# christofw/multipitch_architectures

Measured on NVIDIA B200. Metric: audio_seconds_per_second, higher is better.
Workload: dtype fp16

## Files before the change

include/mpa.h:

```cpp
#ifndef MPA_H_
#define MPA_H_

#include <stddef.h>
#include <stdint.h>

#ifdef __cplusplus
extern "C" {
#endif

#define MPA_OK 0
#define MPA_ERR_ARG (-1)
#define MPA_ERR_ARCH (-2)
#define MPA_ERR_CUDA (-3)
#define MPA_ERR_WORKSPACE (-4)

#define MPA_ACT_NONE 0
#define MPA_ACT_LRELU 1
#define MPA_ACT_RELU 2
#define MPA_ACT_SIGMOID 3

#define MPA_FMT_F16 0
#define MPA_FMT_BF16 1
#define MPA_FMT_F16X3 2

// ... 112 lines not shown
int mpa_conv_tc_pack_weights_dev(const float* w_dev, void* packed_dev, int Cin, int Cout, int KH, int KW, int fmt, int J,
                                 int transpose_flip, int Cout_total, int co0, void* stream);
typedef struct mpa_pack_job {
  const float* w;
  void* packed;
  int Cin, Cout, KH, KW, fmt, J, transpose_flip, Cout_total, co0;
  int split, C0;
} mpa_pack_job;
int mpa_conv_tc_pack_weights_split_dev(const float* w_dev, void* packed_dev, int Cin, int Cout, int KH, int KW, int fmt, int J,
                                       int transpose_flip, int Cout_total, int co0, int split, int C0, void* stream);
size_t mpa_conv_tc_pack_table_bytes(int n_jobs);
int mpa_conv_tc_pack_table_build(const mpa_pack_job* jobs, int n_jobs, void* table_host);
int mpa_conv_tc_pack_weights_multi(const void* table_dev, int n_jobs, int n_blocks, void* stream);
size_t mpa_conv_tc_ring_packed_bytes(int Cin, int Cout, int KH, int KW, int J);
int mpa_conv_tc_ring_pack_weights(const float* w_host, void* packed_host, int Cin, int Cout, int KH, int KW, int fmt, int J);
int mpa_conv_tc_pool_f16(const mpa_conv_tc_desc* desc, void* stream);
int mpa_pool_time_res_cp8(const void* y_cp8, const void* res_cp8, void* out_cp8, int n_patches, int C, int T, int F,
                          int pitch, int pf, int pt, int k, int fmt, int ncs_y, int ncs_res, int ncs_out, void* stream);
int mpa_maxpool2x2_cp8(const void* in_cp8, void* out_cp8, int n, int C, int T, int F, int pitch_in, int pf_in,
                       int pt_in, int ncs_in, int pitch_out, int pf_out, int pt_out, int ncs_out, int fmt, void* stream);
int mpa_upsample2x_cp8(const void* low_cp8, void* out_cp8, int n, int C, int Tl, int Fl, int pitch_l, int pf_l, int pt_l,
                       int ncs_l, int Ts, int Fs, int pitch_s, int pf_s, int pt_s, int ncs_out, int fmt, void* stream);
int mpa_nchw_to_cp8(const float* x, void* out_cp8, int B, int C, int T, int F, int pitch, int pf, int pt, int fmt,
                    int ncs_out, void* stream);
int mpa_nchw_to_cp8_strided(const float* x, void* out_cp8, int B, int C, int T, int Fs, int F, int stride, int offset, int pitch,
                            int pf, int pt, int fmt, int ncs_out, void* stream);
int mpa_cp8_to_nchw(const void* in_cp8, float* out, int B, int C, int T, int F, int pitch, int pf, int pt, int fmt,
                    int ncs_in, void* stream);

int mpa_head_tail_cp8(const void* x_cp8, const float* w3, const float* b3, const float* w40, const float* b40,
                      const float* w43, const float* b43, float* out, int B, int C1, int T, int Fo, int C2, int C3,
// ... 167 lines not shown
```

multipitch_architectures_b200/csrc/conv_tc.cu:

```cuda
#include "common.cuh"
#include <cuda.h>
#include <cuda_fp16.h>
#include <vector>
#include <string.h>
#include <math.h>

namespace mpa {

constexpr int kStageMMAs = 8;
constexpr int kATileBytes = 2 * 128 * 16;
constexpr int kAStageBytes = kStageMMAs * kATileBytes;
constexpr int kMaxAStages = 5;
constexpr int kNumBStages = 2;
constexpr int kMaxBStages = 8;
constexpr int kThreads = 320;
constexpr int kMaxRingS = 24;
constexpr int kMaxRingB = 8;
constexpr int kMaxGrid = 160;
constexpr int kEpiPitch = 40;
constexpr unsigned long long kWaitTimeoutNs = 4000000000ull;

struct ConvTcParams {
  const uint8_t* in_edge;
  const uint8_t* in_stream;
// ... 140 lines not shown

struct UnitInfo {
  int b, seg, t0;
  bool first_in_seg;
};
__device__ __forceinline__ UnitInfo decode_unit(const ConvTcParams& p, int u) {
  UnitInfo ui;
  ui.b = u / p.groups_per_patch;
  int g = u - ui.b * p.groups_per_patch;
  ui.seg = 0;
  if (g >= p.seg_groups[0]) { g -= p.seg_groups[0]; ui.seg = 1; }
  ui.t0 = p.y_lo[ui.seg] + g * p.J * p.R;
  ui.first_in_seg = (g == 0);
  return ui;
}
__device__ __forceinline__ void unit_range(const ConvTcParams& p, int& u_begin, int& u_end, int& u_first_real) {
  const long long U = p.n_units;
  u_first_real = (int)(U * blockIdx.x / gridDim.x);
  u_end = (int)(U * (blockIdx.x + 1) / gridDim.x);
  u_begin = u_first_real;
  if (p.pool && u_first_real < u_end && !decode_unit(p, u_first_real).first_in_seg) u_begin = u_first_real - 1;
}
__device__ __forceinline__ const uint8_t* in_row_ptr(const ConvTcParams& p, int b, int row, long long& chunk_stride) {
  if (row < p.in_e || row >= p.T - p.in_e) {
    const int idx = row < p.in_e ? row : row - (p.T - 2 * p.in_e);
    chunk_stride = p.in_edge_chunk_stride;
    return p.in_edge + (long long)b * p.in_edge_patch_stride + (long long)idx * p.P * 16;
  }
  chunk_stride = p.in_stream_chunk_stride;
  return p.in_stream + ((long long)b * p.in_stream_patch_rows + row) * p.P * 16;
}
__device__ __forceinline__ uint8_t* out_row_ptr(const ConvTcParams& p, int b, int row, long long& chunk_stride) {
  if (row < p.out_e || row >= p.T - p.out_e) {
    const int idx = row < p.out_e ? row : row - (p.T - 2 * p.out_e);
    chunk_stride = p.out_edge_chunk_stride;
    return p.out_edge + (long long)b * p.out_edge_patch_stride + (long long)idx * p.P * 16;
// ... 28 lines not shown
    }
  } else {
    __half2* cm = reinterpret_cast<__half2*>(&c);
    const __half2* rm = reinterpret_cast<const __half2*>(&r);
#pragma unroll
    for (int e = 0; e < 4; ++e) {
      float2 a = __half22float2(cm[e]), b2 = __half22float2(rm[e]);
      cm[e] = __floats2half2_rn(a.x + b2.x, a.y + b2.y);
    }
  }
  return c;
}

template <bool X3>
__device__ __forceinline__ void epilogue_role(const ConvTcParams& p, uint32_t tmem_base, uint16_t* epi_smem, uint64_t* acc_full, uint64_t* acc_empty,
                                              int u_begin, int u_end, int u_first_real) {
  const int warp = threadIdx.x >> 5, lane = threadIdx.x & 31;
  {
    const int quad = warp & 3;
    const int m = quad * 32 + lane;
    const int j = m / p.Cout, co = m - j * p.Cout;
    const bool row_valid = (j < p.J);
    const float bias = row_valid ? p.bias[co] : 0.f;
    const float inv_scale = (X3 && row_valid) ? p.inv_scale[co] : 1.f;
    constexpr int n_parts = X3 ? 2 : 1;
    const float act_slope = p.act == MPA_ACT_NONE ? 1.f : p.act == MPA_ACT_RELU ? 0.f : p.act_param;
    const bool fast_act = p.act != MPA_ACT_SIGMOID && act_slope >= 0.f && act_slope <= 1.f;
    const int NCoP = n_parts * p.NCo;
    const bool staged = ((p.Cout & 7) == 0);
    const int ewarp = warp - 2;
    const int ehalf = ewarp >> 2;
    const int etid = threadIdx.x - 64;
    uint16_t* stile = epi_smem + ewarp * (32 * kEpiPitch);
    int grp_j[4], grp_plane[4];
#pragma unroll
    for (int k = 0; k < 4; ++k) {
      const int mg = quad * 32 + k * 8;
      grp_j[k] = mg / p.Cout;
      grp_plane[k] = (mg - grp_j[k] * p.Cout) >> 3;
    }
    const size_t plane_elems = (p.out_mode == 0) ? (size_t)p.TP_out * p.P * 8 : (p.out_mode == 2) ? (size_t)p.TP_out * p.P2 * 8 : (size_t)p.T_out * p.F_out * 8;
    const int row_pitch = (p.out_mode == 0) ? p.P : (p.out_mode == 2) ? p.P2 : p.F_out;
    const size_t ring_row_bytes = (size_t)NCoP * p.P * 16;
    uint8_t* ring_cta = p.pool ? p.ring + (size_t)blockIdx.x * 2 * p.J * ring_row_bytes : nullptr;
    uint32_t k_unit = 0;
    for (int u = u_begin; u < u_end; ++u, ++k_unit) {
      const UnitInfo ui = decode_unit(p, u);
      const int b = ui.b, t0 = ui.t0;
      const int y_hi = p.y_hi[ui.seg];
      const int t = t0 + j;
      const uint32_t buf = k_unit & 1u, acc_par = (k_unit >> 1) & 1u;
      uint8_t* ring_bank = p.pool ? ring_cta + (size_t)(k_unit & 1u) * p.J * ring_row_bytes : nullptr;
      mbar_wait(&acc_full[buf], acc_par);
      tc_fence_after();
      uint16_t* out_b = p.out + (size_t)b * p.out_patch_stride;
      for (int c0 = ehalf * 32; c0 < p.N; c0 += 64) {
        const int n = c0 + lane;
        int rr = 0, nn = n;
        if (p.R > 1) { rr = n / p.P; nn = n - rr * p.P; }
        int fo = nn - p.pf;
// ... 156 lines not shown
              *reinterpret_cast<uint4*>(op) = c;
            } else {
              long long ocs;
              uint8_t* op = out_row_ptr(p, b, tz, ocs);
              *reinterpret_cast<uint4*>(op + (long long)ck * ocs + (size_t)(p.pf + f) * 16) = c;
            }
          }
        }
        epi_bar_sync();
      }
    }
  }
}

template <bool X3>
__global__ void __launch_bounds__(kThreads, 1) conv_tc_kernel(const __grid_constant__ ConvTcParams p) {
  extern __shared__ __align__(1024) uint8_t smem[];
  const int slab_plane_bytes = p.slab_px * 16;
  const int bstage_bytes = min(p.G, p.NC) * slab_plane_bytes + p.bpad;
  const int kNumAStages = p.a_stages;
  uint8_t* a_smem = smem;
  uint8_t* b_smem = smem + kNumAStages * kAStageBytes;
  const int nbs = p.b_stages;
  uint64_t* bars = reinterpret_cast<uint64_t*>(b_smem + nbs * bstage_bytes);
  uint64_t* a_full = bars;
  uint64_t* a_empty = bars + kMaxAStages;
  uint64_t* b_full = bars + 2 * kMaxAStages;
  uint64_t* b_empty = b_full + kMaxBStages;
  uint64_t* acc_full = b_empty + kMaxBStages;
  uint64_t* acc_empty = acc_full + 2;
  uint32_t* tmem_slot = reinterpret_cast<uint32_t*>(acc_empty + 2);
// ... 21 lines not shown
    for (int i = threadIdx.x; i < nbs * bstage_bytes / 16; i += kThreads) reinterpret_cast<uint4*>(b_smem)[i] = make_uint4(0, 0, 0, 0);
    asm volatile("fence.proxy.async.shared::cta;" ::: "memory");
  }
  if (warp == 1) {
    asm volatile("tcgen05.alloc.cta_group::1.sync.aligned.shared::cta.b32 [%0], %1;" ::"r"(smem_u32(tmem_slot)), "r"(512u));
    asm volatile("tcgen05.relinquish_alloc_permit.cta_group::1.sync.aligned;");
  }
  tc_fence_before();
  __syncthreads();
  tc_fence_after();
  const uint32_t tmem_base = *tmem_slot;

  const int ph = p.KH / 2, pw = p.KW / 2;
  const int rows_in = p.KH + p.J - 1;
  constexpr int n_parts = X3 ? 2 : 1;
  int u_begin, u_end, u_first_real;
  unit_range(p, u_begin, u_end, u_first_real);

  if (warp == 0) {
    {
      int a_stage = 0, b_stage = 0;
      uint32_t a_phase = 0, b_phase = 0;
      if (lane == 0 && p.resident && u_begin < u_end) {
        const int spr = (p.mmas_per_row + kStageMMAs - 1) / kStageMMAs;
        for (int r = 0; r < rows_in; ++r)
          for (int m0 = 0; m0 < p.mmas_per_row; m0 += kStageMMAs) {
            const int nm = min(kStageMMAs, p.mmas_per_row - m0), idx = r * spr + m0 / kStageMMAs;
            mbar_expect_tx(&a_full[idx], (uint32_t)(nm * kATileBytes));
            bulk_g2s(a_smem + idx * kAStageBytes, p.w + ((size_t)r * p.mmas_per_row + m0) * kATileBytes, (uint32_t)(nm * kATileBytes), &a_full[idx]);
          }
      }
      __syncwarp();
      for (int u = u_begin; u < u_end; ++u) {
        const UnitInfo ui = decode_unit(p, u);
        for (int r = 0; r < rows_in; ++r) {
          const int row = ui.t0 - ph + r;
          if (p.R == 1 && (row < 0 || row >= p.T)) continue;
          for (int part = 0; part < n_parts; ++part) {
           for (int gi = 0; gi < p.n_groups; ++gi) {
            const int planes = min(p.G, p.NC - gi * p.G);
            uint8_t* dst = b_smem + b_stage * bstage_bytes;
            if (p.tma) {
              if (lane == 0) {
                mbar_wait(&b_empty[b_stage], b_phase ^ 1);
                mbar_expect_tx(&b_full[b_stage], (uint32_t)(min(p.G, p.NC) * slab_plane_bytes));
                asm volatile(
                    "cp.async.bulk.tensor.4d.shared::cluster.global.tile.mbarrier::complete_tx::bytes [%0], [%1, {%2, %3, %4, %5}], [%6];" ::"r"(
// ... 40 lines not shown
            const int n_tiles = (X3 && part == 0) ? 2 * p.mmas_per_row : (gi == p.n_groups - 1 ? p.mmas_per_row : (gi + 1) * (p.G / 2) * p.KW) - q0;
            const uint8_t* wrow = p.w + ((size_t)r * p.tiles_per_row + (part ? 2 * p.mmas_per_row : 0) + q0) * kATileBytes;
            for (int m0 = 0; m0 < n_tiles; m0 += kStageMMAs) {
              const int nm = min(kStageMMAs, n_tiles - m0);
              if (lane == 0) {
                mbar_wait(&a_empty[a_stage], a_phase ^ 1);
                mbar_expect_tx(&a_full[a_stage], (uint32_t)(nm * kATileBytes));
                bulk_g2s(a_smem + a_stage * kAStageBytes, wrow + (size_t)m0 * kATileBytes, (uint32_t)(nm * kATileBytes), &a_full[a_stage]);
              }
              if (++a_stage == kNumAStages) { a_stage = 0; a_phase ^= 1; }
            }
           }
          }
        }
      }
    }
    __syncwarp();
  } else if (warp == 1) {
    {
      const uint32_t tmem_u = __shfl_sync(0xffffffffu, tmem_base, 0);
      int a_stage = 0, b_stage = 0;
      uint32_t a_phase = 0, b_phase = 0;
      constexpr uint32_t kDescHi = (128u >> 4) | (1u << 14);
      constexpr uint32_t kALoFixed = ((128u * 16u) >> 4) << 16;
      const uint32_t asm16 = smem_u32(a_smem) >> 4, bsm16 = smem_u32(b_smem) >> 4, bst16 = (uint32_t)bstage_bytes >> 4;
      uint32_t k_unit = 0;
      const int spr = (p.mmas_per_row + kStageMMAs - 1) / kStageMMAs;
      if (p.resident && u_begin < u_end)
        for (int i = 0; i < rows_in * spr; ++i) mbar_wait(&a_full[i], 0);
      for (int u = u_begin; u < u_end; ++u, ++k_unit) {
        const UnitInfo ui = decode_unit(p, u);
        const uint32_t buf = k_unit & 1u, acc_par = (k_unit >> 1) & 1u;
        mbar_wait(&acc_empty[buf], acc_par ^ 1);
        tc_fence_after();
        const uint32_t tmem_d = tmem_u + buf * 256;
        uint32_t accum = 0;
        for (int r = 0; r < rows_in; ++r) {
          const int row = ui.t0 - ph + r;
          if (p.R == 1 && (row < 0 || row >= p.T)) continue;
          for (int part = 0; part < n_parts; ++part) {
          for (int gi = 0; gi < p.n_groups; ++gi) {
          const int q0 = gi * (p.G / 2) * p.KW;
          const int n_tiles = (X3 && part == 0) ? 2 * p.mmas_per_row : (gi == p.n_groups - 1 ? p.mmas_per_row : (gi + 1) * (p.G / 2) * p.KW) - q0;
          mbar_wait(&b_full[b_stage], b_phase);
// ... 20 lines not shown
              if (!p.resident) tc_commit(&a_empty[a_stage]);
            }
            __syncwarp();
            accum = 1;
            if (!p.resident && ++a_stage == kNumAStages) { a_stage = 0; a_phase ^= 1; }
          }
          if (elect_one_sync()) tc_commit(&b_empty[b_stage]);
          __syncwarp();
          if (++b_stage == nbs) { b_stage = 0; b_phase ^= 1; }
          }
          }
        }
        if (elect_one_sync()) tc_commit(&acc_full[buf]);
        __syncwarp();
      }
    }
    __syncwarp();
  } else {
    epilogue_role<X3>(p, tmem_base, epi_smem, acc_full, acc_empty, u_begin, u_end, u_first_real);
  }
  tc_fence_before();
  __syncthreads();
  if (warp == 1) {
    tc_fence_after();
    asm volatile("tcgen05.dealloc.cta_group::1.sync.aligned.b32 %0, %1;" ::"r"(tmem_base), "r"(512u));
  }
}

template <int Q, int BSTEP>
__device__ __forceinline__ void issue_tile(uint32_t tmem_d, uint32_t a_lo, uint32_t a_hi, uint32_t b_lo, uint32_t b_hi, uint32_t idesc, uint32_t first) {
  tc_mma_f16(tmem_d, ((uint64_t)a_hi << 32) | (uint64_t)a_lo, ((uint64_t)b_hi << 32) | (uint64_t)b_lo, idesc, first ? 0u : 1u);
#pragma unroll
  for (int q = 1; q < Q; ++q)
    tc_mma_f16(tmem_d, ((uint64_t)a_hi << 32) | (uint64_t)(a_lo + (uint32_t)q * 16u), ((uint64_t)b_hi << 32) | (uint64_t)(b_lo + (uint32_t)(q * BSTEP)), idesc, 1u);
}
__device__ __forceinline__ void ring_group(const ConvTcParams& p, int g, int& Q, int& planes, int& chunk0) {
  if (g < p.NC / 2) { Q = p.KW; planes = 2; chunk0 = 2 * g; }
  else { Q = (p.KW + 1) / 2; planes = 1; chunk0 = p.NC - 1; }
}

__global__ void __launch_bounds__(kThreads, 1) conv_tc_ring_kernel(const ConvTcParams p) {
  extern __shared__ __align__(1024) uint8_t smem[];
  const int slab_plane_bytes = p.slab_px * 16;
  const int bstage_bytes = 2 * slab_plane_bytes;
  const int S = p.ring_S, NB = p.ring_nb;
  uint8_t* ring = smem;
  uint8_t* b_smem = smem + p.ring_b_off;
  uint64_t* bars = reinterpret_cast<uint64_t*>(smem + p.ring_bar_off);
  uint64_t* w_full = bars;
  uint64_t* w_empty = bars + kMaxRingS;
  uint64_t* b_full = bars + 2 * kMaxRingS;
  uint64_t* b_empty = b_full + kMaxRingB;
  uint64_t* acc_full = b_empty + kMaxRingB;
  uint64_t* acc_empty = acc_full + 2;
  uint32_t* tmem_slot = reinterpret_cast<uint32_t*>(acc_empty + 2);
  uint32_t* btab = reinterpret_cast<uint32_t*>(smem + p.btab_off);
// ... 8 lines not shown
  }
  if (warp == 1) {
    asm volatile("tcgen05.alloc.cta_group::1.sync.aligned.shared::cta.b32 [%0], %1;" ::"r"(smem_u32(tmem_slot)), "r"(512u));
    asm volatile("tcgen05.relinquish_alloc_permit.cta_group::1.sync.aligned;");
  }
  tc_fence_before();
  __syncthreads();
  tc_fence_after();
  const uint32_t tmem_base = *tmem_slot;

  const int ph = p.KH / 2, pw = p.KW / 2;
  const int rows_in = p.KH + p.J - 1;
  const int NG = (p.NC + 1) / 2;
  const int G8 = p.Cout >> 3;
  const int n_kh = p.KH + 2 * (p.J - 1);
  int u_begin, u_end, u_first_real;
  unit_range(p, u_begin, u_end, u_first_real);

  if (warp == 0) {
    if (lane == 0) {
      uint32_t n_piece = 0;
      int b_stage = 0;
      uint32_t b_phase = 0;
      for (int u = u_begin; u < u_end; ++u) {
        const UnitInfo ui = decode_unit(p, u);
        const int r_first = max(0, ph - ui.t0), r_last = min(rows_in - 1, p.T - 1 - ui.t0 + ph);
        size_t g_off = 0;
        for (int g = 0; g < NG; ++g) {
          int Q, planes, chunk0;
          ring_group(p, g, Q, planes, chunk0);
          const uint32_t row_bytes = (uint32_t)Q * 256u;
          const uint8_t* wg = p.w + g_off;
          for (int kh = r_first - (p.J - 1); kh <= r_last; ++kh, ++n_piece) {
            const int pos = S - 1 - (int)(n_piece % (uint32_t)S);
            const uint32_t round = n_piece / (uint32_t)S;
            const bool mirror = pos <= p.J - 2;
            mbar_wait(&w_empty[pos], (round & 1u) ^ 1u);
            const bool mir = mirror;
// ... 12 lines not shown
            if (kh >= r_first) {
              const int row = ui.t0 - ph + kh;
              mbar_wait(&b_empty[b_stage], b_phase ^ 1);
              mbar_expect_tx(&b_full[b_stage], (uint32_t)(planes * slab_plane_bytes));
              long long cs;
              const uint8_t* bsrc = in_row_ptr(p, ui.b, row, cs) - pw * 16 + (long long)chunk0 * cs;
              uint8_t* bdst = b_smem + b_stage * bstage_bytes;
              for (int c = 0; c < planes; ++c)
                bulk_g2s(bdst + c * slab_plane_bytes, bsrc + (long long)c * cs, (uint32_t)slab_plane_bytes, &b_full[b_stage]);
              if (++b_stage == NB) { b_stage = 0; b_phase ^= 1; }
            }
          }
          g_off += (size_t)n_kh * G8 * row_bytes;
        }
      }
    }
    __syncwarp();
  } else if (warp == 1) {
    {
      const uint32_t tmem_u = __shfl_sync(0xffffffffu, tmem_base, 0);
      uint32_t n_piece = 0;
      int b_stage = 0;
      uint32_t b_phase = 0;
      const uint32_t kDescHiB = (128u >> 4) | (1u << 14);
      const uint32_t kDescHiA = ((uint32_t)p.ring_sbo >> 4) | (1u << 14);
      constexpr uint32_t kALoFixed = (128u >> 4) << 16;
      const uint32_t ring16 = smem_u32(ring) >> 4, ps16 = (uint32_t)p.ring_ps >> 4;
      const uint32_t bsm16 = smem_u32(b_smem) >> 4, bst16 = (uint32_t)bstage_bytes >> 4;
      const uint32_t plane16 = (uint32_t)slab_plane_bytes >> 4;
      uint32_t k_unit = 0;
      for (int u = u_begin; u < u_end; ++u, ++k_unit) {
        const UnitInfo ui = decode_unit(p, u);
        const int r_first = max(0, ph - ui.t0), r_last = min(rows_in - 1, p.T - 1 - ui.t0 + ph);
        const uint32_t buf = k_unit & 1u, acc_par = (k_unit >> 1) & 1u;
        mbar_wait(&acc_empty[buf], acc_par ^ 1);
        tc_fence_after();
        const uint32_t tmem_d = tmem_u + buf * 256;
        uint32_t first = 1;
        for (int g = 0; g < NG; ++g) {
          const bool pair = g < p.NC / 2;
          const int Q = pair ? p.KW : (p.KW + 1) / 2;
          const uint32_t b_lo_fixed = pair ? (plane16 << 16) : (1u << 16);
          for (int kh = r_first - (p.J - 1); kh <= r_last; ++kh, ++n_piece) {
            const int pos = S - 1 - (int)(n_piece % (uint32_t)S);
            mbar_wait(&w_full[pos], (n_piece / (uint32_t)S) & 1u);
// ... 13 lines not shown
                             p.idesc, (q == 0 && first) ? 0u : 1u);
              }
              tc_commit(&b_empty[b_stage]);
              tc_commit(&w_empty[S - 1 - (int)(n_old % (uint32_t)S)]);
              if (kh == r_last)
                for (int jj = p.J - 2; jj >= 0; --jj) tc_commit(&w_empty[S - 1 - (int)((n_piece - (uint32_t)jj) % (uint32_t)S)]);
            }
            __syncwarp();
            first = 0;
            if (++b_stage == NB) { b_stage = 0; b_phase ^= 1; }
          }
        }
        if (elect_one_sync()) tc_commit(&acc_full[buf]);
        __syncwarp();
      }
    }
  } else {
    epilogue_role<false>(p, tmem_base, epi_smem, acc_full, acc_empty, u_begin, u_end, u_first_real);
  }
  tc_fence_before();
  __syncthreads();
  if (warp == 1) {
    tc_fence_after();
    asm volatile("tcgen05.dealloc.cta_group::1.sync.aligned.b32 %0, %1;" ::"r"(tmem_base), "r"(512u));
  }
}

static inline int j_blocks(int Cout) { return Cout >= 128 ? 1 : 128 / Cout; }
static inline int mmas_per_row(int NC, int KW) { return (NC / 2) * KW + ((NC & 1) ? (KW + 1) / 2 : 0); }

static inline uint16_t f32_to_f16_rne(float f) {
  uint32_t x;
  memcpy(&x, &f, 4);
// ... 706 lines not shown
              const int co = g8 * 8 + row;
              for (int e = 0; e < 8; ++e) {
                const int ci = c * 8 + e;
                if (ci >= Cin) continue;
                const float wv = w[(((size_t)co * Cin + ci) * KH + kh) * KW + df];
                o[g_off + ((((size_t)khi * G8 + g8) * Q + q) * 2 + ks) * 64 + row * 8 + e] = fmt == MPA_FMT_BF16 ? f32_to_bf16_rne(wv) : f32_to_f16_rne(wv);
              }
            }
          }
    }
    g_off += (size_t)n_kh * G8 * Q * 128;
  }
  return MPA_OK;
}

static int launch_conv_tc(ConvTcParams& p, int Cin, cudaStream_t stream, int* grid_out) {
  p.mmas_per_row = mmas_per_row(p.NC, p.KW);
  p.slab_px = (p.N + 2 * (p.KW / 2) + 1 + 7) / 8 * 8;
  if (p.R < 1) p.R = 1;
  if (p.Rs < 1) p.Rs = 1;
  p.tma = 0;
  p.tma_c0 = 0;
  const bool tma_ok = !p.x3 && !p.ring_on && p.in_e == p.T && tensor_map_encoder();
  if (tma_ok && (p.Rs > 1 || p.R > 1) && p.KW == 1) {
    p.tma = 1;
    p.slab_px = p.N;
  } else if (tma_ok && p.R == 1 && p.Rs == 1 && p.NC >= 2 && p.slab_px <= 128) {
    p.tma = 2;
    p.tma_c0 = -2 * (p.KW / 2);
  }
  p.bpad = p.tma ? 128 : 0;
  size_t smem = 0;
  if (p.x3) {
    MPA_REQUIRE(!p.ring_on, "conv_tc: the ring main loop has no split-precision variant");
    MPA_REQUIRE((p.Cout & 7) == 0, "conv_tc(fp16x3): Cout must be a multiple of 8 (got %d)", p.Cout);
    p.inv_scale = (const float*)(p.w + (size_t)3 * (p.KH + p.J - 1) * p.mmas_per_row * kATileBytes);
  }
  if (p.ring_on) {
// ... 73 lines not shown
  MPA_REQUIRE(smem <= 227 * 1024, "conv_tc: needs %zu B of shared memory (Cin=%d pitch=%d)", smem, Cin, p.P);
  {
    static unsigned char flags_tile[64], flags_ring[64], flags_x3[64];
    cudaError_t e = p.ring_on ? opt_in_max_smem(conv_tc_ring_kernel, flags_ring)
                    : p.x3    ? opt_in_max_smem(conv_tc_kernel<true>, flags_x3)
                              : opt_in_max_smem(conv_tc_kernel<false>, flags_tile);
    if (e != cudaSuccess) {
      set_error("conv_tc: cudaFuncSetAttribute: %s", cudaGetErrorString(e));
      return MPA_ERR_CUDA;
    }
  }
  int dev = 0, sms = 148;
  cudaGetDevice(&dev);
  cudaDeviceGetAttribute(&sms, cudaDevAttrMultiProcessorCount, dev);
  if (sms > kMaxGrid) sms = kMaxGrid;
  const int grid = p.n_units < sms ? p.n_units : sms;
  if (grid_out) *grid_out = grid;
  if (p.ring_on)
    conv_tc_ring_kernel<<<grid, kThreads, smem, stream>>>(p);
  else if (p.x3)
    conv_tc_kernel<true><<<grid, kThreads, smem, stream>>>(p);
  else
    conv_tc_kernel<false><<<grid, kThreads, smem, stream>>>(p);
  MPA_CHECK_LAUNCH("conv_tc");
  return MPA_OK;
}

int mpa_conv_tc_f16(const void* in_cp8, const void* w_packed, const float* bias, void* out, int out_mode, int sub_stride,
                    int sub_offset, int n_patches, int Cin, int Cout, int T, int F, int KH, int KW, int pitch, int pf, int pt,
                    long long in_patch_stride_rows, int in_nc_stride, int out_nc_stride, int J, int row0, int n_rows, int act,
                    float act_param, int fmt, void* stream) {
  MPA_CHECK_ARCH();
  MPA_REQUIRE(in_cp8 && w_packed && bias && out && n_patches > 0, "conv_tc: null argument");
  MPA_REQUIRE(Cout > 0 && Cout <= 128 && Cin > 0, "conv_tc: Cout must be in 1..128 (got %d)", Cout);
  MPA_REQUIRE((KH & 1) && (KW & 1), "conv_tc: odd kernel sizes only");
  MPA_REQUIRE(fmt == MPA_FMT_F16 || fmt == MPA_FMT_BF16 || fmt == MPA_FMT_F16X3, "conv_tc: fmt must be MPA_FMT_F16, MPA_FMT_BF16 or MPA_FMT_F16X3");
  const bool x3 = fmt == MPA_FMT_F16X3;
  MPA_REQUIRE(!x3 || in_patch_stride_rows <= 0, "conv_tc(fp16x3): the streaming input goes through mpa_conv_tc_pool_f16");
// ... 65 lines not shown
    p.R = 256 / pitch;
    p.Rs = p.J;
    p.N = p.R * pitch;
  }
  p.n_seg = 1;
  p.y_lo[0] = p.z_lo[0] = row0;
  p.y_hi[0] = p.z_hi[0] = row0 + p.T_out;
  p.seg_groups[0] = (p.T_out + p.J * p.R - 1) / (p.J * p.R);
  p.seg_groups[1] = 0;
  p.groups_per_patch = p.seg_groups[0];
  p.n_units = n_patches * p.groups_per_patch;
  p.act = act;
  p.act_param = act_param;
  const uint32_t f = (fmt == MPA_FMT_BF16) ? 1u : 0u;
  p.idesc = (1u << 4) | (f << 7) | (f << 10) | ((uint32_t)(p.N >> 3) << 17) | ((uint32_t)(128 >> 4) << 24);
  return launch_conv_tc(p, Cin, (cudaStream_t)stream, nullptr);
}

size_t mpa_conv_tc_pool_workspace(int Cout, int pitch, int J) {
  if (Cout <= 0 || Cout > 128 || pitch <= 0) return 0;
  if (J <= 0) J = j_blocks(Cout);
  return (size_t)kMaxGrid * 2 * J * ((Cout + 7) / 8) * pitch * 16;
}

size_t mpa_conv_tc_pool_workspace_fmt(int Cout, int pitch, int J, int fmt) {
  return mpa_conv_tc_pool_workspace(Cout, pitch, J) * (fmt == MPA_FMT_F16X3 ? 2 : 1);
}

int mpa_conv_tc_pool_f16(const mpa_conv_tc_desc* d, void* stream) {
  MPA_CHECK_ARCH();
  MPA_REQUIRE(d && d->w_packed && d->bias && d->workspace && d->n_patches > 0, "conv_tc_pool: null argument");
  MPA_REQUIRE(d->Cout > 0 && d->Cout <= 64 && (d->Cout & 7) == 0 && d->Cin > 0, "conv_tc_pool: Cout must be a multiple of 8, <= 64 (got %d)", d->Cout);
  MPA_REQUIRE((d->KH & 1) && (d->KW & 1), "conv_tc_pool: odd kernel sizes only");
  MPA_REQUIRE(d->fmt == MPA_FMT_F16 || d->fmt == MPA_FMT_BF16 || d->fmt == MPA_FMT_F16X3, "conv_tc_pool: fmt must be MPA_FMT_F16, MPA_FMT_BF16 or MPA_FMT_F16X3");
  const int pitch = d->pitch, KW = d->KW, F = d->F, pf = d->pf, T = d->T;
  MPA_REQUIRE(pitch >= 16 && pitch <= 256 && pitch % 16 == 0, "conv_tc_pool: row pitch %d must be a multiple of 16 (<= 256)", pitch);
  MPA_REQUIRE(pf >= KW / 2 && pitch - F >= KW / 2 && pitch >= pf + F, "conv_tc_pool: pitch %d / left pad %d too small for F=%d KW=%d", pitch, pf, F, KW);
  const int J = d->J > 0 ? d->J : j_blocks(d->Cout);
  MPA_REQUIRE(J >= 2 && J * d->Cout <= 128, "conv_tc_pool: needs 2 <= J and J*Cout <= 128");
  MPA_REQUIRE(d->in_e == T || (d->in_e >= 0 && 2 * d->in_e <= T), "conv_tc_pool: in_e must be T or <= T/2");
  MPA_REQUIRE(d->out_e == T || (d->out_e >= 0 && 2 * d->out_e <= T), "conv_tc_pool: out_e must be T or <= T/2");
  MPA_REQUIRE((d->in_e == 0 || d->in_edge) && (d->in_e == T || d->in_stream), "conv_tc_pool: missing input plane");
  MPA_REQUIRE((d->out_e == 0 || d->out_edge) && (d->out_e == T || d->out_stream), "conv_tc_pool: missing output plane");
  MPA_REQUIRE(d->n_seg == 1 || d->n_seg == 2, "conv_tc_pool: 1 or 2 row segments");
  ConvTcParams p;
  memset(&p, 0, sizeof(p));
  p.in_edge = (const uint8_t*)d->in_edge;
  p.in_stream = (const uint8_t*)d->in_stream;
  p.in_edge_patch_stride = d->in_edge_patch_stride;
  p.in_edge_chunk_stride = d->in_edge_chunk_stride;
  p.in_stream_chunk_stride = d->in_stream_chunk_stride;
  p.in_stream_patch_rows = d->in_stream_patch_rows;
  p.in_e = d->in_e;
  p.out_edge = (uint8_t*)d->out_edge;
  p.out_stream = (uint8_t*)d->out_stream;
  p.out_edge_patch_stride = d->out_edge_patch_stride;
  p.out_edge_chunk_stride = d->out_edge_chunk_stride;
  p.out_stream_chunk_stride = d->out_stream_chunk_stride;
  p.out_stream_patch_rows = d->out_stream_patch_rows;
  p.out_e = d->out_e;
// ... 32 lines not shown
    p.z_lo[s] = d->z_lo[s];
    p.z_hi[s] = d->z_hi[s];
    p.y_lo[s] = d->z_lo[s] > 0 ? d->z_lo[s] - 1 : 0;
    p.y_hi[s] = d->z_hi[s] < T ? d->z_hi[s] + 1 : T;
    p.seg_groups[s] = (p.y_hi[s] - p.y_lo[s] + J - 1) / J;
    p.groups_per_patch += p.seg_groups[s];
  }
  MPA_REQUIRE(d->n_seg == 1 || p.y_hi[0] <= p.y_lo[1], "conv_tc_pool: row segments overlap");
  p.n_units = d->n_patches * p.groups_per_patch;
  p.ring = (uint8_t*)d->workspace;
  MPA_REQUIRE(d->ws_bytes >= mpa_conv_tc_pool_workspace_fmt(d->Cout, pitch, J, d->fmt), "conv_tc_pool: workspace too small (%zu B)", d->ws_bytes);
  p.act = d->act;
  p.act_param = d->act_param;
  const uint32_t f = (d->fmt == MPA_FMT_BF16) ? 1u : 0u;
  p.idesc = (1u << 4) | (f << 7) | (f << 10) | ((uint32_t)(p.N >> 3) << 17) | ((uint32_t)(128 >> 4) << 24);
  return launch_conv_tc(p, d->Cin, (cudaStream_t)stream, nullptr);
}

int mpa_pool_time_res_cp8(const void* y_cp8, const void* res_cp8, void* out_cp8, int n_patches, int C, int T, int F, int pitch, int pf,
                          int pt, int k, int fmt, int ncs_y, int ncs_res, int ncs_out, void* stream) {
  MPA_CHECK_ARCH();
  MPA_REQUIRE(y_cp8 && out_cp8 && n_patches > 0 && C > 0 && k >= 1 && (k & 1) && pitch >= pf + F, "pool_time_res_cp8: bad argument");
  const int NCk = (C + 7) / 8;
  if (ncs_y <= 0) ncs_y = NCk;
  if (ncs_res <= 0) ncs_res = NCk;
  if (ncs_out <= 0) ncs_out = NCk;
  long long total = (long long)n_patches * NCk * T * F;
  if (fmt == MPA_FMT_F16X3) {
    if (ncs_y == NCk) ncs_y = 2 * NCk;
    if (ncs_res == NCk) ncs_res = 2 * NCk;
    if (ncs_out == NCk) ncs_out = 2 * NCk;
// ... 123 lines not shown
```

multipitch_architectures_b200/engine.py:

```python
import numpy as np
import torch

from . import _lib, ops
from .libdl.nn_models import _exec
from .libdl.nn_models.basic_cnns import basic_cnn_segm_sigmoid, deep_cnn_segm_sigmoid

CONTEXT = 75
HALF = CONTEXT // 2


class CnnStreamEngine:

    def __init__(self, model, chunk=646, compression=10.0, fused=True, dedup=True, ring=False, split_head=True):
        if not isinstance(model, (basic_cnn_segm_sigmoid, deep_cnn_segm_sigmoid)):
            raise TypeError('CnnStreamEngine serves the CNN / DCNN / DRCNN family')
        self.model, self.chunk, self.compression = model, int(chunk), float(compression)
        self.dev = next(model.parameters()).device
        if self.dev.type != 'cuda':
            raise _lib.MpaError('the engine needs the model on a CUDA (sm_100a) device')
        if not _exec.tc_eligible(model, model.n_bins_in):
            raise _lib.MpaError("CnnStreamEngine needs precision 'fp16', 'bf16' or 'fp16x3' and <=128 channels per layer; "
                                "use predict_patchwise for the fp32 path")
        self.fmt = ops.fmt_of(model.precision)
        self.x3 = self.fmt == ops.FMT_F16X3
# ... 111 lines not shown
        R = N + T - 1
        e = self._edges()
        streams, edges, ws = self._virtual_buffers(R)
        packed, biases = [], []
        for i, (name, conv) in enumerate(self.blocks):
            w = conv.weight
            if self.x3:
                wp, b = _exec.block_operands(cache, name, conv, self.fmt, self.dev, C if i == 0 else self.C0, self.C0)
            else:
                wp = cache.get(f'{name}:wtc{self.fmt}:{int(self.ring)}', [w], lambda: ops.conv_tc_pack(w, self.dev, self.fmt, ring=self.ring))
                b = conv.bias
            packed.append(wp)
            biases.append(b)
        plane_stream = plane

        def run(i, src, dst, n, segments, tag, out_split=0):
            cin = C if i == 0 else self.C0
            self._timed(tag, lambda: ops.conv_tc_pool(src, dst, packed[i], biases[i], n, cin, self.C0, F, (self.KH, self.KW), self.pitch, self.pf,
                                                      segments, self.residual and i > 0, ops.ACT_LRELU, a, self.fmt, ws, ring=self.ring,
                                                      out_split=out_split),
                        work=n * sum(hi_ - lo_ for lo_, hi_ in segments))
        for i, ei in enumerate(e):
            if ei == T:
                break
            src = ops.VRows(R, 0, stream=plane_stream if i == 0 else streams[i - 1])
            run(i, src, ops.VRows(R, 0, stream=streams[i]), 1, [(ei, R - ei)], 'conv_tc_stream')
        direct = _exec.head_tc_supported(m, T, F) and T == m.conv3[0].kernel_size[0]
        result = torch.empty(hi - lo, F // 3, dtype=torch.float32, device=self.dev) if direct else None
        outs = []
        for i0 in range(lo, hi, self.chunk):
            n = min(self.chunk, hi - i0)
            prev = ops.VRows(T, 0, stream=plane_stream, row0=i0)
            for i, ei in enumerate(e):
                dst = ops.VRows(T, ei, edge=edges[i], stream=streams[i], row0=i0)
                segs = [(0, ei), (T - ei, T)] if ei < T else [(0, T)]
                last = i == len(e) - 1
                run(i, prev, dst, n, segs, 'conv_tc_first' if i == 0 else 'conv_tc', out_split=self.split if (last and self.split) else 0)
                prev = dst
            if self.split:
                sb = edges[-1]
                zc = ops.CP8(n, self.split * self.C0, T, F // self.split, sb.shape[3], 8, 1, self.dev, buf=sb, fmt=self.fmt)
            else:
                zc = ops.CP8(n, self.C0, T, F, self.pitch, self.pf, 1, self.dev, buf=edges[-1], fmt=self.fmt)
            y = self._timed('head', lambda: _exec.head_tc(cache, m, zc, a, split=self.split, pool=self._head_pool,
                                                          out=result[i0 - lo:i0 - lo + n] if direct else None))
            if not direct:
                outs.append(y.reshape(n, -1))
        if hi == lo:
            return torch.empty(0, 0, dtype=torch.float32, device=self.dev)
        if direct:
            return result
        return outs[0] if len(outs) == 1 else torch.cat(outs, 0)
# ... 61 lines not shown
```

multipitch_architectures_b200/ops.py:

```python
import torch

from . import _lib
from ._lib import call, stream_ptr

ACT_NONE, ACT_LRELU, ACT_RELU, ACT_SIGMOID = 0, 1, 2, 3


def _f32(t):
    if not t.is_cuda:
        raise _lib.MpaError('libmpa operators take CUDA tensors only (no CPU path exists)')
    if t.dtype != torch.float32:
        raise _lib.MpaError(f'expected float32 tensor, got {t.dtype}')
    return t


def pack_conv_weight(w):
    Cout, Cin, KH, KW = w.shape
    CoutPad = (Cout + 15) // 16 * 16
    p = torch.zeros(Cin, KH * KW, CoutPad, dtype=torch.float32, device=w.device)
    p[:, :, :Cout] = w.detach().float().permute(1, 2, 3, 0).reshape(Cin, KH * KW, Cout)
    return p.contiguous()


def layernorm_cf(x, w, b, eps=1e-5, gamma_log=0.0):
# ... 361 lines not shown
        ed = (0, 0, 0)
        if self.edge is not None:
            n, NC, RE = self.edge.shape[0], self.edge.shape[1], self.edge.shape[2]
            ed = (self.edge.data_ptr() + row, NC * RE * row, RE * row)
        st = (0, 0)
        if self.stream is not None:
            st = (self.stream.data_ptr() + (1 + self.row0) * row, self.stream.shape[1] * row)
        return ed, st


def conv_tc_pool_workspace(Cout, pitch, device, J=0, fmt=FMT_F16):
    n = _lib.lib().mpa_conv_tc_pool_workspace_fmt(Cout, pitch, J, fmt)
    return torch.empty(n, dtype=torch.uint8, device=device)


def conv_tc_pool(src, dst, w_packed, bias, n_patches, Cin, Cout, F, ksize, pitch, pf, segments, residual, act, act_param, fmt, workspace, J=0,
                 ring=False, out_split=0):
    d = ConvTcDesc()
    (d.in_edge, d.in_edge_patch_stride, d.in_edge_chunk_stride), (d.in_stream, d.in_stream_chunk_stride) = src.fields(pitch)
    d.in_stream_patch_rows, d.in_e = src.patch_rows, src.e
    d.out_split = int(out_split)
    (d.out_edge, d.out_edge_patch_stride, d.out_edge_chunk_stride), (d.out_stream, d.out_stream_chunk_stride) = \
        dst.fields(dst.edge.shape[3] if out_split else pitch)
    d.out_stream_patch_rows, d.out_e = dst.patch_rows, dst.e
    d.w_packed, d.bias = w_packed.data_ptr(), bias.data_ptr()
    d.n_patches, d.Cin, d.Cout, d.T, d.F, d.KH, d.KW, d.pitch, d.pf, d.J = n_patches, Cin, Cout, src.T, F, ksize[0], ksize[1], pitch, pf, J
    d.n_seg = len(segments)
    for i, (lo, hi) in enumerate(segments):
        d.z_lo[i], d.z_hi[i] = lo, hi
    d.residual, d.act, d.act_param, d.fmt = int(bool(residual)), act, float(act_param), fmt
    d.weights_layout = 1 if ring else 0
    d.workspace, d.ws_bytes = workspace.data_ptr(), workspace.numel()
    rc = _lib.lib().mpa_conv_tc_pool_f16(_ct.byref(d), stream_ptr())
    if rc != 0:
        raise _lib.MpaError(f'mpa_conv_tc_pool_f16 failed ({rc}): {_lib.last_error()}')
    return dst


_ZERO_ROWS = {}


def _zero_row(device, nbytes):
    key = str(device)
    z = _ZERO_ROWS.get(key)
    if z is None or z.numel() < nbytes:
        z = torch.zeros(max(nbytes, 16 * 256 * 16), dtype=torch.uint8, device=device)
        _ZERO_ROWS[key] = z
    return z
# ... 139 lines not shown
```

Baseline: 737.7.

## Fuse streaming-row conv launches into the edge-row conv kernel launch

Instead of launching a separate conv_tc kernel for each layer's streaming middle rows before the edge-row convolutions, the stream row set is passed as a second parameter block and its work units are prepended to the same grid's unit range. Producer, MMA and epilogue roles iterate over both unit sets with a shared accumulator counter. This removes several small kernel launches and the associated tail idle time, at the cost of disabling the TMA path when fused and adding extra kernel parameters.

```diff
diff --git a/include/mpa.h b/include/mpa.h
--- a/include/mpa.h
+++ b/include/mpa.h
@@ -150,7 +150,7 @@
 int mpa_conv_tc_pack_weights_multi(const void* table_dev, int n_jobs, int n_blocks, void* stream);
 size_t mpa_conv_tc_ring_packed_bytes(int Cin, int Cout, int KH, int KW, int J);
 int mpa_conv_tc_ring_pack_weights(const float* w_host, void* packed_host, int Cin, int Cout, int KH, int KW, int fmt, int J);
-int mpa_conv_tc_pool_f16(const mpa_conv_tc_desc* desc, void* stream);
+int mpa_conv_tc_pool_f16(const mpa_conv_tc_desc* desc, const mpa_conv_tc_desc* stream_desc, void* stream);
 int mpa_pool_time_res_cp8(const void* y_cp8, const void* res_cp8, void* out_cp8, int n_patches, int C, int T, int F,
                           int pitch, int pf, int pt, int k, int fmt, int ncs_y, int ncs_res, int ncs_out, void* stream);
 int mpa_maxpool2x2_cp8(const void* in_cp8, void* out_cp8, int n, int C, int T, int F, int pitch_in, int pf_in,
diff --git a/multipitch_architectures_b200/csrc/conv_tc.cu b/multipitch_architectures_b200/csrc/conv_tc.cu
--- a/multipitch_architectures_b200/csrc/conv_tc.cu
+++ b/multipitch_architectures_b200/csrc/conv_tc.cu
@@ -178,12 +178,18 @@
   ui.first_in_seg = (g == 0);
   return ui;
 }
-__device__ __forceinline__ void unit_range(const ConvTcParams& p, int& u_begin, int& u_end, int& u_first_real) {
-  const long long U = p.n_units;
-  u_first_real = (int)(U * blockIdx.x / gridDim.x);
-  u_end = (int)(U * (blockIdx.x + 1) / gridDim.x);
-  u_begin = u_first_real;
-  if (p.pool && u_first_real < u_end && !decode_unit(p, u_first_real).first_in_seg) u_begin = u_first_real - 1;
+__device__ __forceinline__ void unit_range(const ConvTcParams& p, const ConvTcParams& ps, int (&u_begin)[2], int (&u_end)[2], int (&u_first_real)[2]) {
+  const int Us = ps.n_units;
+  const long long U = (long long)Us + p.n_units;
+  const int first = (int)(U * blockIdx.x / gridDim.x), end = (int)(U * (blockIdx.x + 1) / gridDim.x);
+  int begin = first;
+  if (p.pool && first < end && !(first < Us ? decode_unit(ps, first) : decode_unit(p, first - Us)).first_in_seg) begin = first - 1;
+  u_begin[0] = min(begin, Us);
+  u_end[0] = min(end, Us);
+  u_first_real[0] = first;
+  u_begin[1] = max(begin - Us, 0);
+  u_end[1] = max(end - Us, 0);
+  u_first_real[1] = max(first - Us, 0);
 }
 __device__ __forceinline__ const uint8_t* in_row_ptr(const ConvTcParams& p, int b, int row, long long& chunk_stride) {
   if (row < p.in_e || row >= p.T - p.in_e) {
@@ -242,7 +248,7 @@
 
 template <bool X3>
 __device__ __forceinline__ void epilogue_role(const ConvTcParams& p, uint32_t tmem_base, uint16_t* epi_smem, uint64_t* acc_full, uint64_t* acc_empty,
-                                              int u_begin, int u_end, int u_first_real) {
+                                              int u_begin, int u_end, int u_first_real, uint32_t& k_unit) {
   const int warp = threadIdx.x >> 5, lane = threadIdx.x & 31;
   {
     const int quad = warp & 3;
@@ -271,7 +277,6 @@
     const int row_pitch = (p.out_mode == 0) ? p.P : (p.out_mode == 2) ? p.P2 : p.F_out;
     const size_t ring_row_bytes = (size_t)NCoP * p.P * 16;
     uint8_t* ring_cta = p.pool ? p.ring + (size_t)blockIdx.x * 2 * p.J * ring_row_bytes : nullptr;
-    uint32_t k_unit = 0;
     for (int u = u_begin; u < u_end; ++u, ++k_unit) {
       const UnitInfo ui = decode_unit(p, u);
       const int b = ui.b, t0 = ui.t0;
@@ -458,7 +463,8 @@
 }
 
 template <bool X3>
-__global__ void __launch_bounds__(kThreads, 1) conv_tc_kernel(const __grid_constant__ ConvTcParams p) {
+__global__ void __launch_bounds__(kThreads, 1) conv_tc_kernel(const __grid_constant__ ConvTcParams p,
+                                                                const __grid_constant__ ConvTcParams ps) {
   extern __shared__ __align__(1024) uint8_t smem[];
   const int slab_plane_bytes = p.slab_px * 16;
   const int bstage_bytes = min(p.G, p.NC) * slab_plane_bytes + p.bpad;
@@ -510,14 +516,15 @@
   const int ph = p.KH / 2, pw = p.KW / 2;
   const int rows_in = p.KH + p.J - 1;
   constexpr int n_parts = X3 ? 2 : 1;
-  int u_begin, u_end, u_first_real;
-  unit_range(p, u_begin, u_end, u_first_real);
+  int u_begin[2], u_end[2], u_first_real[2];
+  unit_range(p, ps, u_begin, u_end, u_first_real);
+  const bool any_units = u_begin[0] < u_end[0] || u_begin[1] < u_end[1];
 
   if (warp == 0) {
     {
       int a_stage = 0, b_stage = 0;
       uint32_t a_phase = 0, b_phase = 0;
-      if (lane == 0 && p.resident && u_begin < u_end) {
+      if (lane == 0 && p.resident && any_units) {
         const int spr = (p.mmas_per_row + kStageMMAs - 1) / kStageMMAs;
         for (int r = 0; r < rows_in; ++r)
           for (int m0 = 0; m0 < p.mmas_per_row; m0 += kStageMMAs) {
@@ -527,6 +534,7 @@
           }
       }
       __syncwarp();
+      auto units = [&](const ConvTcParams& p, int u_begin, int u_end) {
       for (int u = u_begin; u < u_end; ++u) {
         const UnitInfo ui = decode_unit(p, u);
         for (int r = 0; r < rows_in; ++r) {
@@ -597,6 +605,9 @@
           }
         }
       }
+      };
+      units(ps, u_begin[0], u_end[0]);
+      units(p, u_begin[1], u_end[1]);
     }
     __syncwarp();
   } else if (warp == 1) {
@@ -609,8 +620,9 @@
       const uint32_t asm16 = smem_u32(a_smem) >> 4, bsm16 = smem_u32(b_smem) >> 4, bst16 = (uint32_t)bstage_bytes >> 4;
       uint32_t k_unit = 0;
       const int spr = (p.mmas_per_row + kStageMMAs - 1) / kStageMMAs;
-      if (p.resident && u_begin < u_end)
+      if (p.resident && any_units)
         for (int i = 0; i < rows_in * spr; ++i) mbar_wait(&a_full[i], 0);
+      auto units = [&](const ConvTcParams& p, int u_begin, int u_end) {
       for (int u = u_begin; u < u_end; ++u, ++k_unit) {
         const UnitInfo ui = decode_unit(p, u);
         const uint32_t buf = k_unit & 1u, acc_par = (k_unit >> 1) & 1u;
@@ -661,10 +673,15 @@
         if (elect_one_sync()) tc_commit(&acc_full[buf]);
         __syncwarp();
       }
+      };
+      units(ps, u_begin[0], u_end[0]);
+      units(p, u_begin[1], u_end[1]);
     }
     __syncwarp();
   } else {
-    epilogue_role<X3>(p, tmem_base, epi_smem, acc_full, acc_empty, u_begin, u_end, u_first_real);
+    uint32_t k_unit = 0;
+    epilogue_role<X3>(ps, tmem_base, epi_smem, acc_full, acc_empty, u_begin[0], u_end[0], u_first_real[0], k_unit);
+    epilogue_role<X3>(p, tmem_base, epi_smem, acc_full, acc_empty, u_begin[1], u_end[1], u_first_real[1], k_unit);
   }
   tc_fence_before();
   __syncthreads();
@@ -686,7 +703,7 @@
   else { Q = (p.KW + 1) / 2; planes = 1; chunk0 = p.NC - 1; }
 }
 
-__global__ void __launch_bounds__(kThreads, 1) conv_tc_ring_kernel(const ConvTcParams p) {
+__global__ void __launch_bounds__(kThreads, 1) conv_tc_ring_kernel(const __grid_constant__ ConvTcParams p, const __grid_constant__ ConvTcParams ps) {
   extern __shared__ __align__(1024) uint8_t smem[];
   const int slab_plane_bytes = p.slab_px * 16;
   const int bstage_bytes = 2 * slab_plane_bytes;
@@ -725,14 +742,15 @@
   const int NG = (p.NC + 1) / 2;
   const int G8 = p.Cout >> 3;
   const int n_kh = p.KH + 2 * (p.J - 1);
-  int u_begin, u_end, u_first_real;
-  unit_range(p, u_begin, u_end, u_first_real);
+  int u_begin[2], u_end[2], u_first_real[2];
+  unit_range(p, ps, u_begin, u_end, u_first_real);
 
   if (warp == 0) {
     if (lane == 0) {
       uint32_t n_piece = 0;
       int b_stage = 0;
       uint32_t b_phase = 0;
+      auto units = [&](const ConvTcParams& p, int u_begin, int u_end) {
       for (int u = u_begin; u < u_end; ++u) {
         const UnitInfo ui = decode_unit(p, u);
         const int r_first = max(0, ph - ui.t0), r_last = min(rows_in - 1, p.T - 1 - ui.t0 + ph);
@@ -775,6 +793,9 @@
           g_off += (size_t)n_kh * G8 * row_bytes;
         }
       }
+      };
+      units(ps, u_begin[0], u_end[0]);
+      units(p, u_begin[1], u_end[1]);
     }
     __syncwarp();
   } else if (warp == 1) {
@@ -790,6 +811,7 @@
       const uint32_t bsm16 = smem_u32(b_smem) >> 4, bst16 = (uint32_t)bstage_bytes >> 4;
       const uint32_t plane16 = (uint32_t)slab_plane_bytes >> 4;
       uint32_t k_unit = 0;
+      auto units = [&](const ConvTcParams& p, int u_begin, int u_end) {
       for (int u = u_begin; u < u_end; ++u, ++k_unit) {
         const UnitInfo ui = decode_unit(p, u);
         const int r_first = max(0, ph - ui.t0), r_last = min(rows_in - 1, p.T - 1 - ui.t0 + ph);
@@ -833,9 +855,14 @@
         if (elect_one_sync()) tc_commit(&acc_full[buf]);
         __syncwarp();
       }
+      };
+      units(ps, u_begin[0], u_end[0]);
+      units(p, u_begin[1], u_end[1]);
     }
   } else {
-    epilogue_role<false>(p, tmem_base, epi_smem, acc_full, acc_empty, u_begin, u_end, u_first_real);
+    uint32_t k_unit = 0;
+    epilogue_role<false>(ps, tmem_base, epi_smem, acc_full, acc_empty, u_begin[0], u_end[0], u_first_real[0], k_unit);
+    epilogue_role<false>(p, tmem_base, epi_smem, acc_full, acc_empty, u_begin[1], u_end[1], u_first_real[1], k_unit);
   }
   tc_fence_before();
   __syncthreads();
@@ -1572,14 +1599,14 @@
   return MPA_OK;
 }
 
-static int launch_conv_tc(ConvTcParams& p, int Cin, cudaStream_t stream, int* grid_out) {
+static int launch_conv_tc(ConvTcParams& p, const ConvTcParams* rows, int Cin, cudaStream_t stream, int* grid_out) {
   p.mmas_per_row = mmas_per_row(p.NC, p.KW);
   p.slab_px = (p.N + 2 * (p.KW / 2) + 1 + 7) / 8 * 8;
   if (p.R < 1) p.R = 1;
   if (p.Rs < 1) p.Rs = 1;
   p.tma = 0;
   p.tma_c0 = 0;
-  const bool tma_ok = !p.x3 && !p.ring_on && p.in_e == p.T && tensor_map_encoder();
+  const bool tma_ok = !rows && !p.x3 && !p.ring_on && p.in_e == p.T && tensor_map_encoder();
   if (tma_ok && (p.Rs > 1 || p.R > 1) && p.KW == 1) {
     p.tma = 1;
     p.slab_px = p.N;
@@ -1683,14 +1710,45 @@
   cudaGetDevice(&dev);
   cudaDeviceGetAttribute(&sms, cudaDevAttrMultiProcessorCount, dev);
   if (sms > kMaxGrid) sms = kMaxGrid;
-  const int grid = p.n_units < sms ? p.n_units : sms;
+  ConvTcParams ps = p;
+  ps.n_units = 0;
+  if (rows) {
+    ps.in_edge = rows->in_edge;
+    ps.in_stream = rows->in_stream;
+    ps.in_edge_patch_stride = rows->in_edge_patch_stride;
+    ps.in_edge_chunk_stride = rows->in_edge_chunk_stride;
+    ps.in_stream_chunk_stride = rows->in_stream_chunk_stride;
+    ps.in_stream_patch_rows = rows->in_stream_patch_rows;
+    ps.in_e = rows->in_e;
+    ps.out_edge = rows->out_edge;
+    ps.out_stream = rows->out_stream;
+    ps.out_edge_patch_stride = rows->out_edge_patch_stride;
+    ps.out_edge_chunk_stride = rows->out_edge_chunk_stride;
+    ps.out_stream_chunk_stride = rows->out_stream_chunk_stride;
+    ps.out_stream_patch_rows = rows->out_stream_patch_rows;
+    ps.out_e = rows->out_e;
+    ps.n_patches = rows->n_patches;
+    ps.T = rows->T;
+    ps.n_seg = rows->n_seg;
+    for (int s = 0; s < 2; ++s) {
+      ps.y_lo[s] = rows->y_lo[s];
+      ps.y_hi[s] = rows->y_hi[s];
+      ps.z_lo[s] = rows->z_lo[s];
+      ps.z_hi[s] = rows->z_hi[s];
+      ps.seg_groups[s] = rows->seg_groups[s];
+    }
+    ps.groups_per_patch = rows->groups_per_patch;
+    ps.n_units = rows->n_units;
+  }
+  const long long units = (long long)p.n_units + ps.n_units;
+  const int grid = units < sms ? (int)units : sms;
   if (grid_out) *grid_out = grid;
   if (p.ring_on)
-    conv_tc_ring_kernel<<<grid, kThreads, smem, stream>>>(p);
+    conv_tc_ring_kernel<<<grid, kThreads, smem, stream>>>(p, ps);
   else if (p.x3)
-    conv_tc_kernel<true><<<grid, kThreads, smem, stream>>>(p);
+    conv_tc_kernel<true><<<grid, kThreads, smem, stream>>>(p, ps);
   else
-    conv_tc_kernel<false><<<grid, kThreads, smem, stream>>>(p);
+    conv_tc_kernel<false><<<grid, kThreads, smem, stream>>>(p, ps);
   MPA_CHECK_LAUNCH("conv_tc");
   return MPA_OK;
 }
@@ -1786,7 +1844,7 @@
   p.act_param = act_param;
   const uint32_t f = (fmt == MPA_FMT_BF16) ? 1u : 0u;
   p.idesc = (1u << 4) | (f << 7) | (f << 10) | ((uint32_t)(p.N >> 3) << 17) | ((uint32_t)(128 >> 4) << 24);
-  return launch_conv_tc(p, Cin, (cudaStream_t)stream, nullptr);
+  return launch_conv_tc(p, nullptr, Cin, (cudaStream_t)stream, nullptr);
 }
 
 size_t mpa_conv_tc_pool_workspace(int Cout, int pitch, int J) {
@@ -1799,8 +1857,7 @@
   return mpa_conv_tc_pool_workspace(Cout, pitch, J) * (fmt == MPA_FMT_F16X3 ? 2 : 1);
 }
 
-int mpa_conv_tc_pool_f16(const mpa_conv_tc_desc* d, void* stream) {
-  MPA_CHECK_ARCH();
+static int pool_params(const mpa_conv_tc_desc* d, ConvTcParams& p) {
   MPA_REQUIRE(d && d->w_packed && d->bias && d->workspace && d->n_patches > 0, "conv_tc_pool: null argument");
   MPA_REQUIRE(d->Cout > 0 && d->Cout <= 64 && (d->Cout & 7) == 0 && d->Cin > 0, "conv_tc_pool: Cout must be a multiple of 8, <= 64 (got %d)", d->Cout);
   MPA_REQUIRE((d->KH & 1) && (d->KW & 1), "conv_tc_pool: odd kernel sizes only");
@@ -1815,7 +1872,6 @@
   MPA_REQUIRE((d->in_e == 0 || d->in_edge) && (d->in_e == T || d->in_stream), "conv_tc_pool: missing input plane");
   MPA_REQUIRE((d->out_e == 0 || d->out_edge) && (d->out_e == T || d->out_stream), "conv_tc_pool: missing output plane");
   MPA_REQUIRE(d->n_seg == 1 || d->n_seg == 2, "conv_tc_pool: 1 or 2 row segments");
-  ConvTcParams p;
   memset(&p, 0, sizeof(p));
   p.in_edge = (const uint8_t*)d->in_edge;
   p.in_stream = (const uint8_t*)d->in_stream;
@@ -1878,7 +1934,24 @@
   p.act_param = d->act_param;
   const uint32_t f = (d->fmt == MPA_FMT_BF16) ? 1u : 0u;
   p.idesc = (1u << 4) | (f << 7) | (f << 10) | ((uint32_t)(p.N >> 3) << 17) | ((uint32_t)(128 >> 4) << 24);
-  return launch_conv_tc(p, d->Cin, (cudaStream_t)stream, nullptr);
+  return MPA_OK;
+}
+
+int mpa_conv_tc_pool_f16(const mpa_conv_tc_desc* d, const mpa_conv_tc_desc* ds, void* stream) {
+  MPA_CHECK_ARCH();
+  ConvTcParams p;
+  int rc = pool_params(d, p);
+  if (rc != MPA_OK) return rc;
+  if (!ds) return launch_conv_tc(p, nullptr, d->Cin, (cudaStream_t)stream, nullptr);
+  ConvTcParams ps;
+  rc = pool_params(ds, ps);
+  if (rc != MPA_OK) return rc;
+  MPA_REQUIRE(ds->w_packed == d->w_packed && ds->bias == d->bias && ds->Cin == d->Cin && ds->Cout == d->Cout && ds->F == d->F && ds->KH == d->KH &&
+                  ds->KW == d->KW && ds->pitch == d->pitch && ds->pf == d->pf && ps.J == p.J && ds->residual == d->residual && ds->act == d->act &&
+                  ds->act_param == d->act_param && ds->fmt == d->fmt && ds->weights_layout == d->weights_layout && ds->workspace == d->workspace &&
+                  ds->out_split == 0,
+              "conv_tc_pool: the stream row set must share the layer (weights, widths, kernel, format, workspace) and have no out_split");
+  return launch_conv_tc(p, &ps, d->Cin, (cudaStream_t)stream, nullptr);
 }
 
 int mpa_pool_time_res_cp8(const void* y_cp8, const void* res_cp8, void* out_cp8, int n_patches, int C, int T, int F, int pitch, int pf,
diff --git a/multipitch_architectures_b200/engine.py b/multipitch_architectures_b200/engine.py
--- a/multipitch_architectures_b200/engine.py
+++ b/multipitch_architectures_b200/engine.py
@@ -149,17 +149,15 @@
             biases.append(b)
         plane_stream = plane
 
-        def run(i, src, dst, n, segments, tag, out_split=0):
+        def run(i, src, dst, n, segments, tag, out_split=0, stream_rows=None):
             cin = C if i == 0 else self.C0
+            work = n * sum(hi_ - lo_ for lo_, hi_ in segments)
+            if stream_rows is not None:
+                work += sum(hi_ - lo_ for lo_, hi_ in stream_rows[3])
             self._timed(tag, lambda: ops.conv_tc_pool(src, dst, packed[i], biases[i], n, cin, self.C0, F, (self.KH, self.KW), self.pitch, self.pf,
                                                       segments, self.residual and i > 0, ops.ACT_LRELU, a, self.fmt, ws, ring=self.ring,
-                                                      out_split=out_split),
-                        work=n * sum(hi_ - lo_ for lo_, hi_ in segments))
-        for i, ei in enumerate(e):
-            if ei == T:
-                break
-            src = ops.VRows(R, 0, stream=plane_stream if i == 0 else streams[i - 1])
-            run(i, src, ops.VRows(R, 0, stream=streams[i]), 1, [(ei, R - ei)], 'conv_tc_stream')
+                                                      out_split=out_split, stream_rows=stream_rows),
+                        work=work)
         direct = _exec.head_tc_supported(m, T, F) and T == m.conv3[0].kernel_size[0]
         result = torch.empty(hi - lo, F // 3, dtype=torch.float32, device=self.dev) if direct else None
         outs = []
@@ -170,7 +168,12 @@
                 dst = ops.VRows(T, ei, edge=edges[i], stream=streams[i], row0=i0)
                 segs = [(0, ei), (T - ei, T)] if ei < T else [(0, T)]
                 last = i == len(e) - 1
-                run(i, prev, dst, n, segs, 'conv_tc_first' if i == 0 else 'conv_tc', out_split=self.split if (last and self.split) else 0)
+                stream_rows = None
+                if i0 == lo and ei < T:
+                    stream_rows = (ops.VRows(R, 0, stream=plane_stream if i == 0 else streams[i - 1]), ops.VRows(R, 0, stream=streams[i]), 1,
+                                   [(ei, R - ei)])
+                run(i, prev, dst, n, segs, 'conv_tc_first' if i == 0 else 'conv_tc', out_split=self.split if (last and self.split) else 0,
+                    stream_rows=stream_rows)
                 prev = dst
             if self.split:
                 sb = edges[-1]
diff --git a/multipitch_architectures_b200/ops.py b/multipitch_architectures_b200/ops.py
--- a/multipitch_architectures_b200/ops.py
+++ b/multipitch_architectures_b200/ops.py
@@ -399,8 +399,8 @@
     return torch.empty(n, dtype=torch.uint8, device=device)
 
 
-def conv_tc_pool(src, dst, w_packed, bias, n_patches, Cin, Cout, F, ksize, pitch, pf, segments, residual, act, act_param, fmt, workspace, J=0,
-                 ring=False, out_split=0):
+def _pool_desc(src, dst, w_packed, bias, n_patches, Cin, Cout, F, ksize, pitch, pf, segments, residual, act, act_param, fmt, workspace, J,
+               ring, out_split):
     d = ConvTcDesc()
     (d.in_edge, d.in_edge_patch_stride, d.in_edge_chunk_stride), (d.in_stream, d.in_stream_chunk_stride) = src.fields(pitch)
     d.in_stream_patch_rows, d.in_e = src.patch_rows, src.e
@@ -416,7 +416,19 @@
     d.residual, d.act, d.act_param, d.fmt = int(bool(residual)), act, float(act_param), fmt
     d.weights_layout = 1 if ring else 0
     d.workspace, d.ws_bytes = workspace.data_ptr(), workspace.numel()
-    rc = _lib.lib().mpa_conv_tc_pool_f16(_ct.byref(d), stream_ptr())
+    return d
+
+
+def conv_tc_pool(src, dst, w_packed, bias, n_patches, Cin, Cout, F, ksize, pitch, pf, segments, residual, act, act_param, fmt, workspace, J=0,
+                 ring=False, out_split=0, stream_rows=None):
+    d = _pool_desc(src, dst, w_packed, bias, n_patches, Cin, Cout, F, ksize, pitch, pf, segments, residual, act, act_param, fmt, workspace, J,
+                   ring, out_split)
+    ds = None
+    if stream_rows is not None:
+        s_src, s_dst, s_n, s_segs = stream_rows
+        ds = _pool_desc(s_src, s_dst, w_packed, bias, s_n, Cin, Cout, F, ksize, pitch, pf, s_segs, residual, act, act_param, fmt, workspace, J,
+                        ring, 0)
+    rc = _lib.lib().mpa_conv_tc_pool_f16(_ct.byref(d), _ct.byref(ds) if ds is not None else None, stream_ptr())
     if rc != 0:
         raise _lib.MpaError(f'mpa_conv_tc_pool_f16 failed ({rc}): {_lib.last_error()}')
     return dst
```

After: 727.2, median of 6. About the same (-1.4%).
